# Giuseppe5/brevitas

Measured on AMD Instinct MI355X. Metric: Gelem/s fused int8 fake-quant fwd+bwd, per-channel, [256,512,56,56], higher is better.
Workload: dtype bf16

## Files before the change

brevitas_amd/csrc/bvq_fakequant.h:

```cpp
#pragma once

#include "bvq_quant_math.h"
#include "bvq_unit_walk.h"
#include "bvq_ties.h"
#include "bvq_sums.h"

namespace bvq {

struct QuantArgs {
  Tiling t;
  const void* x;
  const void* scale;
  const void* zp;
  void* y;
  void* codes;
  const void* g;
  float* ds_part;
  float* dzp_part;
  float* dq_part;
  const float* bounds;
  const void* tie_stat;
  unsigned long long* tie_info;
  unsigned long long* pos_part;
  float qmin, qmax;
  int32_t scale_dtype, zp_dtype;
  int32_t scale_pc, zp_pc;
  int32_t scalar_cast;
  int32_t clamp_ste;
  int32_t out_int;
  int32_t round_mode;
  int32_t pre_relu;
  int32_t codes_dtype;
  uint32_t* arrive;
  uint32_t arrive_per_channel;
  float* dscale_out;
  int32_t gs_scale_dtype, gs_quot_dtype;
  float gs_int_threshold;
  double* shard_msg;
  long long* shard_pos;
  int32_t shard_rank;
  int32_t pre_act;
};

#ifndef BVQ_FWD_UNROLL
#define BVQ_FWD_UNROLL 8
#endif
#ifndef BVQ_BWD_WAVES
#define BVQ_BWD_WAVES 4
#endif
#ifndef BVQ_F16_BWD_DIV
#define BVQ_F16_BWD_DIV 1
#endif
#ifndef BVQ_F16_BWD_PIPE
#define BVQ_F16_BWD_PIPE 1
#endif
#ifndef BVQ_F16_COLS_DIV
#define BVQ_F16_COLS_DIV 1
#endif
#ifndef BVQ_BWD_DEPTH
#define BVQ_BWD_DEPTH 4
#endif
constexpr int kUnroll = BVQ_FWD_UNROLL;
constexpr int kBwdDepth = BVQ_BWD_DEPTH;

template <typename CT>
__device__ __forceinline__ void load_scale_zp(const QuantArgs& a, int32_t channel, float& s, float& z) {
  s = load_scalar_as_f(a.scale, a.scale_dtype, a.scale_pc ? channel : 0);
  z = load_scalar_as_f(a.zp, a.zp_dtype, a.zp_pc ? channel : 0);
  if (a.scalar_cast) {
    if (!a.scale_pc) s = rnd<CT>(s);
    if (!a.zp_pc) z = rnd<CT>(z);
  }
}

template <typename CT, int RM>
__device__ __forceinline__ float do_round(float t, int mode) {
  if constexpr (RM == kAnyRM) {
    return round_any<CT>(t, mode);
  } else {
    return round_op<CT, RM>(t);
  }
}
template <typename CT, int RM>
__device__ __forceinline__ f2 do_round2(f2 t, int mode) {
  if constexpr (RM == kAnyRM) {
    return round_any2<CT>(t, mode);
  } else {
    return round_op2<CT, RM>(t);
  }
}
__device__ __forceinline__ f2 relu2(f2 v) {
  const f2 zero = splat2(0.f);
  return v < zero ? zero : v;
}

struct DivExact {
  float s;
  __device__ __forceinline__ float operator()(float a) const { return a / s; }
  __device__ __forceinline__ f2 operator()(f2 a) const {
    f2 r = {a.x / s, a.y / s};
    return r;
  }
};
struct DivBf16 {
  float r;
  __device__ __forceinline__ float operator()(float a) const { return a * r; }
  __device__ __forceinline__ f2 operator()(f2 a) const { return a * r; }
};

struct DivExactV {
  f2 s;
  __device__ __forceinline__ f2 operator()(f2 a) const {
    f2 r = {a.x / s.x, a.y / s.y};
    return r;
  }
};
struct DivBf16V {
  f2 r;
  __device__ __forceinline__ f2 operator()(f2 a) const { return a * r; }
};

__device__ __forceinline__ bool f16_quot_small(float q) {
  return (__builtin_bit_cast(uint32_t, q) & 0x7fffffffu) - 1u < 0x38810000u - 1u;
}
struct DivF16 {
  float s, r;
  __device__ __forceinline__ float operator()(float a) const {
    float q = a * r;
    if (__builtin_amdgcn_ballot_w64(f16_quot_small(q)) != 0) q = a / s;
    return q;
  }
  __device__ __forceinline__ f2 operator()(f2 a) const {
    f2 q = a * r;
    if (__builtin_amdgcn_ballot_w64(f16_quot_small(q.x) || f16_quot_small(q.y)) != 0) {
      q.x = a.x / s;
      q.y = a.y / s;
    }
    return q;
  }
};
struct DivF16V {
  f2 s, r;
  __device__ __forceinline__ f2 operator()(f2 a) const {
    f2 q = a * r;
    if (__builtin_amdgcn_ballot_w64(f16_quot_small(q.x) || f16_quot_small(q.y)) != 0) {
      q.x = a.x / s.x;
      q.y = a.y / s.y;
    }
    return q;
  }
};
__device__ __forceinline__ float div_refined(float a, float s, float r) {
  const float q0 = a * r;
  const float rem = __builtin_fmaf(-q0, s, a);
  return __builtin_amdgcn_div_fixupf(__builtin_fmaf(rem, r, q0), s, a);
}
struct DivF16R {
  float s, r;
  __device__ __forceinline__ float operator()(float a) const { return div_refined(a, s, r); }
  __device__ __forceinline__ f2 operator()(f2 a) const {
    f2 q = {div_refined(a.x, s, r), div_refined(a.y, s, r)};
    return q;
  }
};
#if BVQ_F16_COLS_DIV
#define BVQ_DIVF16V DivF16RV
#else
#define BVQ_DIVF16V DivF16V
#endif
struct DivF16RV {
  f2 s, r;
  __device__ __forceinline__ f2 operator()(f2 a) const {
    f2 q = {div_refined(a.x, s.x, r.x), div_refined(a.y, s.y, r.y)};
    return q;
  }
};
__device__ __forceinline__ bool f16_scale_ok(float s) {
  const uint32_t sb = __builtin_bit_cast(uint32_t, s);
  return (sb & 0x1fffu) == 0u && s >= 6.103515625e-05f && s <= 16384.f;
}

__device__ __forceinline__ bool bf16_scale_ok(float s) {
  const uint32_t sb = __builtin_bit_cast(uint32_t, s);
  return (sb & 0xffffu) == 0u && s >= 6.103515625e-05f && s <= 16384.f;
}
__device__ __forceinline__ bool zp_is_pos_zero(float z) { return __builtin_bit_cast(uint32_t, z) == 0u; }

struct ColsQuantArgs {
  ColsPlan p;
  const void* x;
  const void* g;
  void* y;
  const void* scale;
  const void* zp;
  float* ds_part;
  unsigned long long* pos_part;
  const void* tie_stat;
  unsigned long long* tie_info;
  int64_t inner;
  int32_t channels;
  float qmin, qmax;
  int32_t scale_dtype, zp_dtype, zp_pc, scalar_cast, clamp_ste, round_mode, pre_relu;
};

template <typename T, int V = elem<T>::vec>
struct ColsLane : ColsPlace {
  static constexpr int VEC = V;
  int32_t ch[VEC];
  f2 s2[VEC / 2], z2[VEC / 2];
  bool fast, zp0;

  __device__ __forceinline__ bool init(const ColsQuantArgs& a, bool team = false) {
    if (!cols_locate(a.p, team, *this)) return false;
    bool ok_fast = true, ok_zp0 = true;
    float sv[VEC], zv[VEC];
#pragma unroll
    for (int k = 0; k < VEC; ++k) {
      const int64_t col = active ? (int64_t)chunk * VEC + k : 0;
      ch[k] = (int32_t)(col / a.inner);
      sv[k] = load_scalar_as_f(a.scale, a.scale_dtype, ch[k]);
      zv[k] = load_scalar_as_f(a.zp, a.zp_dtype, a.zp_pc ? ch[k] : 0);
      if (a.scalar_cast && !a.zp_pc) zv[k] = rnd<T>(zv[k]);
      ok_fast = ok_fast && (elem<T>::id == BVQ_F16 ? f16_scale_ok(sv[k]) : bf16_scale_ok(sv[k]));
      ok_zp0 = ok_zp0 && zp_is_pos_zero(zv[k]);
    }
#pragma unroll
    for (int k = 0; k < VEC / 2; ++k) {
      s2[k] = f2{sv[2 * k], sv[2 * k + 1]};
      z2[k] = f2{zv[2 * k], zv[2 * k + 1]};
    }
    fast = sizeof(T) == 2 && __builtin_amdgcn_ballot_w64(!ok_fast) == 0;
    zp0 = sizeof(T) == 2 && __builtin_amdgcn_ballot_w64(!ok_zp0) == 0;
    return true;
  }
};


static int validate(const bvq_quant_desc* d, bool act = false) {
  if (!d) {
    set_error("null descriptor");
    return BVQ_ERR_INVALID;
  }
  if (d->outer < 0 || d->channels < 1 || d->inner < 0) {
    set_error("bad shape [%lld,%lld,%lld]", (long long)d->outer, (long long)d->channels,
              (long long)d->inner);
    return BVQ_ERR_INVALID;
  }
// ... 97 lines not shown
```

brevitas_amd/csrc/bvq_fakequant_fwd.hip:

```cpp

#include "bvq_act.h"
#include "bvq_fakequant.h"
#include "bvq_stat_epilogue.h"

namespace bvq {

template <typename CT, int RM, bool ZP0, typename Div>
__device__ __forceinline__ float fwd_elem(float xf, const Div& div, float s, float z, float qmin,
                                          float qmax, bool out_int, int mode, float& q_out) {
  float t = rnd<CT>(div(xf));
  t = ZP0 ? t + 0.f : rnd<CT>(t + z);
  t = do_round<CT, RM>(t, mode);
  const float q = clamp_where(t, qmin, qmax);
  q_out = q;
  if (out_int) return q;
  return ZP0 ? rnd<CT>(q * s) : rnd<CT>(rnd<CT>(q - z) * s);
}

template <typename CT, int RM, bool ZP0, typename Div, typename S>
__device__ __forceinline__ f2 fwd_elem2(f2 xf, const Div& div, S s, S z, float qmin, float qmax,
                                        bool out_int, int mode, f2& q_out) {
  f2 t = rnd2<CT>(div(xf));
  t = ZP0 ? t + 0.f : rnd2<CT>(t + z);
  t = do_round2<CT, RM>(t, mode);
  const f2 q = clamp_where2(t, qmin, qmax);
  q_out = q;
  if (out_int) return q;
  return ZP0 ? q * s : rnd2<CT>(q - z) * s;
}

template <int VEC>
__device__ __forceinline__ void store_codes(void* base, int codes_dtype, int64_t off, const float* q) {
  if (codes_dtype == BVQ_CODES_I32) {
    vec_t<int32_t, VEC> cv;
#pragma unroll
    for (int k = 0; k < VEC; ++k) cv.v[k] = (int32_t)q[k];
    store_vec<int32_t, VEC>(reinterpret_cast<int32_t*>(base) + off, cv);
  } else if (codes_dtype == BVQ_CODES_I8) {
    vec_t<int8_t, VEC> cv;
#pragma unroll
    for (int k = 0; k < VEC; ++k) cv.v[k] = (int8_t)(int32_t)q[k];
    store_vec<int8_t, VEC>(reinterpret_cast<int8_t*>(base) + off, cv);
  } else {
    vec_t<uint8_t, VEC> cv;
#pragma unroll
    for (int k = 0; k < VEC; ++k) cv.v[k] = (uint8_t)(int32_t)q[k];
    store_vec<uint8_t, VEC>(reinterpret_cast<uint8_t*>(base) + off, cv);
  }
}

template <typename XT, typename CT, int VEC, int RM, bool NT, bool ZP0, bool PRE, bool NTL = NT, int ACT = 0,
          typename Div>
__device__ __forceinline__ void fwd_unit(const QuantArgs& a, const Unit& u, const Div& div, float s,
                                         float z, float qmin, float qmax) {
  const int lane = threadIdx.x & 63;
  const XT* __restrict__ xp = reinterpret_cast<const XT*>(a.x) + u.base;
  CT* __restrict__ yp = a.y ? reinterpret_cast<CT*>(a.y) + u.base : nullptr;
  void* const cp = a.codes;
  const bool out_int = a.out_int != 0;
  const int mode = a.round_mode;

  ChunkCursor cur;
  cur.init(u, VEC, lane);
  const int64_t total = (int64_t)u.nrows * cur.cpr;
  for (int64_t done = 0; done < total; done += (int64_t)kWave * kUnroll) {
    vec_t<XT, VEC> xv[kUnroll];
    int64_t off[kUnroll];
    bool ok[kUnroll];
#pragma unroll
    for (int j = 0; j < kUnroll; ++j) {
      ok[j] = cur.valid();
      off[j] = cur.offset(u.row_stride, VEC);
      xv[j] = load_vec<XT, VEC, NTL>(xp + (ok[j] ? off[j] : 0));
      cur.next();
    }
#pragma unroll
    for (int j = 0; j < kUnroll; ++j) {
      if (ok[j]) {
        vec_t<CT, VEC> yv;
        float qv[VEC];
        if constexpr (VEC % 2 == 0) {
#pragma unroll
          for (int k = 0; k < VEC; k += 2) {
            f2 xf = widen2<XT>(xv[j].v[k], xv[j].v[k + 1]);
            if constexpr (PRE) xf = relu2(xf);
            if constexpr (ACT != 0) xf = act_rnd2<XT, ACT>(xf);
            f2 q2;
            const f2 r = fwd_elem2<CT, RM, ZP0>(xf, div, s, z, qmin, qmax, out_int, mode, q2);
            pack2<CT>(r, yv.v[k], yv.v[k + 1]);
            qv[k] = q2.x;
            qv[k + 1] = q2.y;
          }
        } else {
#pragma unroll
          for (int k = 0; k < VEC; ++k) {
            float xf = PRE ? relu_f(to_f<XT>(xv[j].v[k])) : to_f<XT>(xv[j].v[k]);
            if constexpr (ACT != 0) xf = act_rnd<XT, ACT>(xf);
            const float r = fwd_elem<CT, RM, ZP0>(xf, div, s, z, qmin, qmax, out_int, mode, qv[k]);
            yv.v[k] = from_f<CT>(r);
          }
        }
        if (yp) store_vec<CT, VEC, NT>(yp + off[j], yv);
        if (cp) store_codes<VEC>(cp, a.codes_dtype, u.base + off[j], qv);
      }
    }
  }
  const int32_t tail = (int32_t)(u.len - (int64_t)cur.cpr * VEC);
  for (int32_t e = lane; e < u.nrows * tail; e += kWave) {
    const int32_t tr = e / tail, tk = e - tr * tail;
    const int64_t i = (int64_t)tr * u.row_stride + (int64_t)cur.cpr * VEC + tk;
    float q;
    float xf = PRE ? relu_f(to_f<XT>(xp[i])) : to_f<XT>(xp[i]);
    if constexpr (ACT != 0) xf = act_rnd<XT, ACT>(xf);
    const float r = fwd_elem<CT, RM, ZP0>(xf, div, s, z, qmin, qmax, out_int, mode, q);
    if (yp) yp[i] = from_f<CT>(r);
    if (cp) store_codes<1>(cp, a.codes_dtype, u.base + i, &q);
  }
}

template <typename XT, typename CT, int VEC, int RM, bool NT, bool NTL = NT, int ACT = 0>
__global__ __launch_bounds__(kBlock) void fakequant_fwd_kernel(QuantArgs a) {
  const Unit u = locate_unit(a.t);
  if (!u.valid) return;
  float s, z;
  load_scale_zp<CT>(a, u.channel, s, z);
  const float qmin = rnd<CT>(a.bounds ? a.bounds[0] : a.qmin), qmax = rnd<CT>(a.bounds ? a.bounds[1] : a.qmax);
  const bool zp0 = sizeof(CT) == 2 && zp_is_pos_zero(z);
#define BVQ_FWD_UNIT(ZP0, PRE, DIV) fwd_unit<XT, CT, VEC, RM, NT, ZP0, PRE, NTL, ACT>(a, u, DIV, s, z, qmin, qmax)
#define BVQ_FWD_PRE(ZP0, DIV)      \
  do {                             \
    if constexpr (ACT != 0)        \
      BVQ_FWD_UNIT(ZP0, false, DIV); \
    else if (a.pre_relu)           \
      BVQ_FWD_UNIT(ZP0, true, DIV); \
    else                           \
      BVQ_FWD_UNIT(ZP0, false, DIV); \
  } while (0)
  if constexpr (elem<CT>::id == BVQ_BF16) {
    if (bf16_scale_ok(s)) {
      const DivBf16 div{1.0f / s};
      if (zp0)
        BVQ_FWD_PRE(true, div);
      else
        BVQ_FWD_PRE(false, div);
      return;
    }
  }
#ifndef BVQ_F16_FWD_EXACT
  if constexpr (elem<CT>::id == BVQ_F16) {
    if (f16_scale_ok(s)) {
      const DivF16R div{s, 1.0f / s};
      if (zp0)
        BVQ_FWD_PRE(true, div);
      else
        BVQ_FWD_PRE(false, div);
      return;
    }
  }
#endif
  const DivExact div{s};
  if constexpr (sizeof(CT) == 2) {
    if (zp0) {
      BVQ_FWD_PRE(true, div);
      return;
    }
  }
  BVQ_FWD_PRE(false, div);
#undef BVQ_FWD_PRE
#undef BVQ_FWD_UNIT
}


template <typename T>
constexpr int kColsFwdVec = sizeof(T) == 2 ? kColsFwdVec16 : elem<T>::vec;

template <typename T, int RM, bool NT, bool ZP0, bool FAST, bool PRE>
__device__ __forceinline__ void cols_fwd_rows(const ColsQuantArgs& a, const ColsLane<T, kColsFwdVec<T>>& ln, float qmin,
                                              float qmax) {
  constexpr int VEC = kColsFwdVec<T>;
#ifndef BVQ_COLS_FWD_UNROLL
#define BVQ_COLS_FWD_UNROLL 4
#endif
  constexpr int kU = BVQ_COLS_FWD_UNROLL;
  const int64_t nrows = ln.row_end - ln.blk0;
  const uint32_t bytes = (uint32_t)(nrows * a.p.L * (int64_t)sizeof(T));
  const buf_t bx = make_buf(reinterpret_cast<const T*>(a.x) + ln.blk0 * a.p.L, bytes);
  const buf_t by = make_buf(reinterpret_cast<T*>(a.y) + ln.blk0 * a.p.L, bytes);
  const uint32_t step = (uint32_t)((int64_t)a.p.rpp * a.p.L * (int64_t)sizeof(T));
  uint32_t off = (uint32_t)(((int64_t)ln.sub * a.p.L + (int64_t)ln.chunk * VEC) * (int64_t)sizeof(T));
  const int32_t steps = (int32_t)((nrows + a.p.rpp - 1) / a.p.rpp);
  f2 r2[VEC / 2];
#pragma unroll
  for (int k = 0; k < VEC / 2; ++k) r2[k] = f2{1.0f / ln.s2[k].x, 1.0f / ln.s2[k].y};
  const int mode = a.round_mode;
  for (int32_t i = 0; i < steps; i += kU) {
    vec_t<T, VEC> xv[kU];
#pragma unroll
    for (int j = 0; j < kU; ++j) xv[j] = buf_load<T, VEC, NT>(bx, off + (uint32_t)j * step);
#pragma unroll
    for (int j = 0; j < kU; ++j) {
      if (i + j < steps) {
        vec_t<T, VEC> yv;
#pragma unroll
        for (int k = 0; k < VEC; k += 2) {
          f2 xf = widen2<T>(xv[j].v[k], xv[j].v[k + 1]);
          if constexpr (PRE) xf = relu2(xf);
          f2 q2, res;
          if constexpr (FAST && elem<T>::id == BVQ_F16)
            res = fwd_elem2<T, RM, ZP0>(xf, BVQ_DIVF16V{ln.s2[k / 2], r2[k / 2]}, ln.s2[k / 2], ln.z2[k / 2], qmin, qmax, false,
                                        mode, q2);
          else if constexpr (FAST)
            res = fwd_elem2<T, RM, ZP0>(xf, DivBf16V{r2[k / 2]}, ln.s2[k / 2], ln.z2[k / 2], qmin, qmax, false, mode, q2);
          else
            res = fwd_elem2<T, RM, ZP0>(xf, DivExactV{ln.s2[k / 2]}, ln.s2[k / 2], ln.z2[k / 2], qmin, qmax, false, mode, q2);
          pack2<T>(res, yv.v[k], yv.v[k + 1]);
        }
        buf_store<T, VEC, NT>(by, off + (uint32_t)j * step, yv);
      }
    }
    off += (uint32_t)kU * step;
  }
}

template <typename T, int RM, bool NT>
__global__ __launch_bounds__(kBlock) void fakequant_fwd_cols_kernel(ColsQuantArgs a) {
  ColsLane<T, kColsFwdVec<T>> ln;
  if (!ln.init(a) || !ln.active) return;
  const float qmin = rnd<T>(a.qmin), qmax = rnd<T>(a.qmax);
#define BVQ_COLS_FWD(ZP0, FAST)                                \
  do {                                                         \
    if (a.pre_relu)                                            \
      cols_fwd_rows<T, RM, NT, ZP0, FAST, true>(a, ln, qmin, qmax);  \
    else                                                       \
      cols_fwd_rows<T, RM, NT, ZP0, FAST, false>(a, ln, qmin, qmax); \
  } while (0)
  if constexpr (sizeof(T) == 2) {
    if (ln.fast) {
      if (ln.zp0)
        BVQ_COLS_FWD(true, true);
      else
        BVQ_COLS_FWD(false, true);
      return;
    }
    if (ln.zp0) {
      BVQ_COLS_FWD(true, false);
      return;
    }
  }
  BVQ_COLS_FWD(false, false);
#undef BVQ_COLS_FWD
}

constexpr int kFusedSlots = 8;
constexpr int kFusedSliceChunks = 512;
constexpr int kFusedMaxWaves = 8;

struct FusedArgs {
  const void* x;
  void* y;
  void* stat_out;
  void* scale_out;
  int64_t outer, inner;
  int32_t channels;
  int32_t cpr;
  int32_t spr;
  int32_t slices;
  float qmin, qmax, min_val, int_threshold;
  int32_t use_min, scale_dtype, scale_pc, scalar_cast, round_mode, pre_relu;
};

template <typename T>
__device__ __forceinline__ float scale_from_key(uint32_t key, bool use_min, float min_val, float int_threshold,
                                                int scale_dtype, float& stat) {
  if constexpr (elem<T>::id == BVQ_F16)
    stat = (float)__builtin_bit_cast(f16_t, (uint16_t)key);
  else
    stat = __builtin_bit_cast(float, key);
  const float thr = (use_min && stat < min_val) ? min_val : stat;
  float s = thr / int_threshold;
  if (scale_dtype == BVQ_BF16)
    s = rnd<bf16_t>(s);
  else if (scale_dtype == BVQ_F16)
    s = rnd<f16_t>(s);
  return s;
}
template <typename T>
__device__ __forceinline__ void store_stat_scale(void* stat_out, void* scale_out, int scale_dtype, int32_t c,
                                                 float stat, float s) {
  if constexpr (elem<T>::id == BVQ_F32)
    reinterpret_cast<float*>(stat_out)[c] = stat;
  else
    reinterpret_cast<T*>(stat_out)[c] = (T)stat;
  if (scale_dtype == BVQ_F32)
    reinterpret_cast<float*>(scale_out)[c] = s;
  else if (scale_dtype == BVQ_BF16)
    reinterpret_cast<bf16_t*>(scale_out)[c] = (bf16_t)s;
  else
    reinterpret_cast<f16_t*>(scale_out)[c] = (f16_t)s;
}

template <typename T, int RM, bool PRE, typename Div, typename Ok>
__device__ __forceinline__ void fused_quantize(const vec_t<T, elem<T>::vec> (&xv)[kFusedSlots], const Ok& ok,
                                               T* __restrict__ yp, int lane, const Div& div, float s,
                                               float qmin, float qmax, int mode) {
  constexpr int VEC = elem<T>::vec;
  constexpr bool ZP0 = sizeof(T) == 2;
#pragma unroll
  for (int j = 0; j < kFusedSlots; ++j) {
    if (ok[j]) {
      vec_t<T, VEC> yv;
#pragma unroll
      for (int k = 0; k < VEC; k += 2) {
        f2 xf = widen2<T>(xv[j].v[k], xv[j].v[k + 1]);
        if constexpr (PRE) xf = relu2(xf);
        f2 q2;
        const f2 r = fwd_elem2<T, RM, ZP0>(xf, div, s, 0.f, qmin, qmax, false, mode, q2);
        pack2<T>(r, yv.v[k], yv.v[k + 1]);
      }
      store_vec<T, VEC, true>(yp + (int64_t)(lane + kWave * j) * VEC, yv);
    }
  }
}

__global__ void fused_zero_kernel(uint32_t* p, int64_t n) {
  const int64_t i = (int64_t)blockIdx.x * blockDim.x + threadIdx.x;
  if (i < n) p[i] = 0u;
}

__device__ __forceinline__ void fused_slice(const FusedArgs& a, int q, int lane, int& r, int& sl, bool (&ok)[kFusedSlots]) {
  const bool active = q < a.slices;
  r = active ? q / a.spr : 0;
  sl = active ? q - r * a.spr : 0;
  const int nch = active ? (a.cpr - sl * kFusedSliceChunks < kFusedSliceChunks ? a.cpr - sl * kFusedSliceChunks
                                                                              : kFusedSliceChunks)
                         : 0;
#pragma unroll
  for (int j = 0; j < kFusedSlots; ++j) ok[j] = lane + kWave * j < nch;
}

template <typename T>
__device__ __forceinline__ void fused_load(const FusedArgs& a, int32_t c, int r, int sl, const bool (&ok)[kFusedSlots],
                                           int lane, vec_t<T, elem<T>::vec> (&xv)[kFusedSlots]) {
  constexpr int VEC = elem<T>::vec;
  const int64_t base = ((int64_t)r * a.channels + c) * a.inner + (int64_t)sl * kFusedSliceChunks * VEC;
  const T* __restrict__ xp = reinterpret_cast<const T*>(a.x) + base;
#pragma unroll
  for (int j = 0; j < kFusedSlots; ++j)
    xv[j] = load_vec<T, VEC, true>(ok[j] ? xp + (int64_t)(lane + kWave * j) * VEC : reinterpret_cast<const T*>(a.x));
}

struct SlotCount {
  int lane, nch;
  __device__ __forceinline__ bool operator[](int j) const { return lane + kWave * j < nch; }
};
__device__ __forceinline__ void fused_slice(const FusedArgs& a, int q, int lane, int& r, int& sl, SlotCount& ok) {
  const bool active = q < a.slices;
  r = active ? q / a.spr : 0;
  sl = active ? q - r * a.spr : 0;
  const int left = a.cpr - sl * kFusedSliceChunks;
  ok.lane = lane;
  ok.nch = active ? (left < kFusedSliceChunks ? left : kFusedSliceChunks) : 0;
}
template <typename T>
__device__ __forceinline__ void fused_load(const FusedArgs& a, int32_t c, int r, int sl, const SlotCount& ok, int lane,
                                           vec_t<T, elem<T>::vec> (&xv)[kFusedSlots]) {
  constexpr int VEC = elem<T>::vec;
  const int64_t base = ((int64_t)r * a.channels + c) * a.inner + (int64_t)sl * kFusedSliceChunks * VEC;
  const T* __restrict__ xp = reinterpret_cast<const T*>(a.x) + base;
  asm volatile("" : "+v"(lane));
#pragma unroll
  for (int j = 0; j < kFusedSlots; ++j)
    xv[j] = load_vec<T, VEC, true>(xp + (lane + kWave * j < ok.nch ? (uint32_t)(lane + kWave * j) * VEC : 0u));
}

template <typename T, typename Ok>
__device__ __forceinline__ uint32_t fused_key(const FusedArgs& a, const vec_t<T, elem<T>::vec> (&xv)[kFusedSlots],
                                              const Ok& ok) {
  uint32_t m = 0;
#pragma unroll
  for (int j = 0; j < kFusedSlots; ++j) {
    if (ok[j]) {
#pragma unroll
      for (int k = 0; k < elem<T>::vec; ++k) {
        const uint32_t b = a.pre_relu ? pre_abs_bits<T, true>(xv[j].v[k]) : pre_abs_bits<T, false>(xv[j].v[k]);
        m = b > m ? b : m;
      }
    }
  }
  return m;
}
template <typename T, std::enable_if_t<sizeof(T) == 4, int> = 0>
__device__ __forceinline__ uint32_t fused_key(const FusedArgs& a, const vec_t<T, elem<T>::vec> (&xv)[kFusedSlots],
                                              const SlotCount& ok) {
  uint32_t m = 0;
#pragma unroll
  for (int j = 0; j < kFusedSlots; ++j) {
    uint32_t mj = 0;
#pragma unroll
    for (int k = 0; k < elem<T>::vec; ++k) {
      const uint32_t b = a.pre_relu ? pre_abs_bits<T, true>(xv[j].v[k]) : pre_abs_bits<T, false>(xv[j].v[k]);
      mj = b > mj ? b : mj;
    }
    mj = ok[j] ? mj : 0u;
    m = mj > m ? mj : m;
  }
  return m;
}

template <typename T, int RM, typename Ok>
__device__ __forceinline__ void fused_apply(const FusedArgs& a, int32_t c, int r, int sl,
                                            const vec_t<T, elem<T>::vec> (&xv)[kFusedSlots], const Ok& ok,
                                            float s, float qmin, float qmax, int lane) {
  constexpr int VEC = elem<T>::vec;
  const int64_t base = ((int64_t)r * a.channels + c) * a.inner + (int64_t)sl * kFusedSliceChunks * VEC;
  T* __restrict__ yp = reinterpret_cast<T*>(a.y) + base;
  const int mode = a.round_mode;
  if constexpr (elem<T>::id == BVQ_BF16) {
    if (bf16_scale_ok(s)) {
      const DivBf16 div{1.0f / s};
      if (a.pre_relu)
        fused_quantize<T, RM, true>(xv, ok, yp, lane, div, s, qmin, qmax, mode);
      else
        fused_quantize<T, RM, false>(xv, ok, yp, lane, div, s, qmin, qmax, mode);
      return;
    }
  }
  if constexpr (elem<T>::id == BVQ_F16) {
    if (f16_scale_ok(s)) {
      const DivF16R div{s, 1.0f / s};
      if (a.pre_relu)
        fused_quantize<T, RM, true>(xv, ok, yp, lane, div, s, qmin, qmax, mode);
      else
        fused_quantize<T, RM, false>(xv, ok, yp, lane, div, s, qmin, qmax, mode);
      return;
    }
  }
  const DivExact div{s};
  if (a.pre_relu)
    fused_quantize<T, RM, true>(xv, ok, yp, lane, div, s, qmin, qmax, mode);
  else
    fused_quantize<T, RM, false>(xv, ok, yp, lane, div, s, qmin, qmax, mode);
}

template <typename T, int RM>
__device__ __forceinline__ void fused_channel(const FusedArgs& a, int32_t c, int r, int sl, const bool (&ok)[kFusedSlots],
                                              float qmin, float qmax, int wave, int lane, int nwaves,
                                              uint32_t* sh_max, uint32_t& sh_stat) {
  vec_t<T, elem<T>::vec> xv[kFusedSlots];
  fused_load<T>(a, c, r, sl, ok, lane, xv);
  const uint32_t m = wave_max_u32(fused_key<T>(a, xv, ok));
  if (lane == 0) sh_max[wave] = m;
  __syncthreads();
  if (threadIdx.x == 0) {
    uint32_t bm = 0;
    for (int w = 0; w < nwaves; ++w) bm = sh_max[w] > bm ? sh_max[w] : bm;
    sh_stat = bm;
  }
  __syncthreads();
  float stat;
  float s = scale_from_key<T>(sh_stat, a.use_min, a.min_val, a.int_threshold, a.scale_dtype, stat);
  if (threadIdx.x == 0) store_stat_scale<T>(a.stat_out, a.scale_out, a.scale_dtype, c, stat, s);
  if (a.scalar_cast && !a.scale_pc) s = rnd<T>(s);
  fused_apply<T, RM>(a, c, r, sl, xv, ok, s, qmin, qmax, lane);
}

template <typename T, int RM>
__global__ __launch_bounds__(kFusedMaxWaves * kWave) void fused_absmax_fakequant_kernel(FusedArgs a) {
  __shared__ uint32_t sh_max[kFusedMaxWaves];
  __shared__ uint32_t sh_stat;
  const int lane = threadIdx.x & 63;
  const int wave = __builtin_amdgcn_readfirstlane((int)(threadIdx.x >> 6));
  const int nwaves = (int)(blockDim.x >> 6);
  int r, sl;
  bool ok[kFusedSlots];
  fused_slice(a, wave, lane, r, sl, ok);
  const float qmin = rnd<T>(a.qmin), qmax = rnd<T>(a.qmax);
  for (int32_t c = blockIdx.x; c < a.channels; c += gridDim.x)
    fused_channel<T, RM>(a, c, r, sl, ok, qmin, qmax, wave, lane, nwaves, sh_max, sh_stat);
}

struct FusedListArgs {
  FusedArgs a[BVQ_WEIGHT_LIST_MAX];
  int32_t start[BVQ_WEIGHT_LIST_MAX + 1];
  int32_t n;
};
static_assert(sizeof(FusedListArgs) <= 4096, "kernel arguments are limited to 4 KiB");

template <typename T, int RM>
__global__ __launch_bounds__(kFusedMaxWaves * kWave) void fused_list_fakequant_kernel(FusedListArgs la) {
  __shared__ uint32_t sh_max[kFusedMaxWaves];
  __shared__ uint32_t sh_stat;
  const int lane = threadIdx.x & 63;
  const int wave = __builtin_amdgcn_readfirstlane((int)(threadIdx.x >> 6));
  const int nwaves = (int)(blockDim.x >> 6);
  int p = -1, r = 0, sl = 0;
  bool ok[kFusedSlots];
  float qmin = 0.f, qmax = 0.f;
  for (int32_t pair = blockIdx.x; pair < la.start[la.n]; pair += gridDim.x) {
    if (p < 0 || pair >= la.start[p + 1]) {
      if (p < 0) p = 0;
      while (p + 1 < la.n && pair >= la.start[p + 1]) ++p;
      fused_slice(la.a[p], wave, lane, r, sl, ok);
      qmin = rnd<T>(la.a[p].qmin);
      qmax = rnd<T>(la.a[p].qmax);
    }
    fused_channel<T, RM>(la.a[p], pair - la.start[p], r, sl, ok, qmin, qmax, wave, lane, nwaves, sh_max, sh_stat);
  }
}


constexpr int kClusterWaves = 16;
constexpr int kClusterMaxMembers = kWave;
constexpr uint32_t kClusterTag = 0x80000000u;
constexpr uint64_t kClusterBudgetTicks = 200000;
enum { kClusterAuto = 0, kClusterWalk = 1, kClusterOneShot = 2 };

struct ClusterArgs {
  FusedArgs f;
  ScaleEpilogue ep;
  void* stat_out;
  int32_t in_dtype;
  uint32_t* key;
  uint32_t* dep;
  uint32_t* fallbacks;
  int32_t members, nclusters, force_fallback;
#ifdef BVQ_CLUSTER_STAMPS
  uint64_t* stamps;
#endif
};

constexpr int kClusterStamps = 6;
#ifdef BVQ_CLUSTER_STAMPS
#define BVQ_CLUSTER_STAMP(k) \
  do {                       \
    if (wave == 0) tk[k] = __builtin_amdgcn_s_memrealtime(); \
  } while (0)
#else
#define BVQ_CLUSTER_STAMP(k) \
  do {                       \
  } while (0)
#endif

__device__ __forceinline__ uint32_t cluster_wave_max(uint32_t v) {
#define BVQ_DPP_MAX(ctrl)                                                                       \
  do {                                                                                          \
    const uint32_t o = (uint32_t)__builtin_amdgcn_update_dpp(0, (int)v, ctrl, 0xf, 0xf, false); \
    v = o > v ? o : v;                                                                          \
  } while (0)
  BVQ_DPP_MAX(0xB1);
  BVQ_DPP_MAX(0x4E);
  BVQ_DPP_MAX(0x141);
  BVQ_DPP_MAX(0x140);
#undef BVQ_DPP_MAX
  const uint32_t a = (uint32_t)__builtin_amdgcn_readlane((int)v, 0), b = (uint32_t)__builtin_amdgcn_readlane((int)v, 16);
  const uint32_t c = (uint32_t)__builtin_amdgcn_readlane((int)v, 32), d = (uint32_t)__builtin_amdgcn_readlane((int)v, 48);
  const uint32_t ab = a > b ? a : b, cd = c > d ? c : d;
  return ab > cd ? ab : cd;
}

template <typename T>
__device__ __forceinline__ uint32_t cluster_fallback_key(const FusedArgs& a, int32_t c, int wave, int lane) {
  constexpr int VEC = elem<T>::vec;
  uint32_t fm = 0;
  for (int q = wave; q < a.slices; q += kClusterWaves) {
    const int fr = q / a.spr, fsl = q - fr * a.spr;
    const int left = a.cpr - fsl * kFusedSliceChunks;
    const int nch = left < kFusedSliceChunks ? left : kFusedSliceChunks;
    const T* xp = reinterpret_cast<const T*>(a.x) + ((int64_t)fr * a.channels + c) * a.inner +
                  (int64_t)fsl * kFusedSliceChunks * VEC;
#pragma clang loop unroll(disable)
    for (int i = lane; i < nch; i += kWave) {
      const vec_t<T, VEC> u = load_vec<T, VEC, false>(xp + (int64_t)i * VEC);
#pragma unroll
      for (int k = 0; k < VEC; ++k) {
        const uint32_t b = a.pre_relu ? pre_abs_bits<T, true>(u.v[k]) : pre_abs_bits<T, false>(u.v[k]);
        fm = b > fm ? b : fm;
      }
    }
  }
  return cluster_wave_max(fm);
}

template <typename T, int RM>
__global__ __launch_bounds__(kClusterWaves * kWave, 8) void cluster_absmax_fakequant_kernel(ClusterArgs ca) {
  constexpr int VEC = elem<T>::vec;
  __shared__ uint32_t sh_max[kClusterWaves];
  __shared__ uint32_t sh_stat, sh_ok;
  const FusedArgs& a = ca.f;
  const int lane = threadIdx.x & 63;
  const int wave = __builtin_amdgcn_readfirstlane((int)(threadIdx.x >> 6));
  const int32_t members = ca.members;
  const int32_t member = (int32_t)blockIdx.x % members, cluster = (int32_t)blockIdx.x / members;
  int r, sl;
  SlotCount ok;
  fused_slice(a, member * kClusterWaves + wave, lane, r, sl, ok);
  const float qmin = rnd<T>(a.qmin), qmax = rnd<T>(a.qmax);
  int32_t c = cluster;
  if (c >= a.channels) return;
#ifdef BVQ_CLUSTER_STAMPS
  uint64_t tk[kClusterStamps] = {};
#endif
  BVQ_CLUSTER_STAMP(0);
  vec_t<T, VEC> xv[kFusedSlots];
  fused_load<T>(a, c, r, sl, ok, lane, xv);
  for (; c < a.channels; c += ca.nclusters) {
    const uint32_t m = cluster_wave_max(fused_key<T>(a, xv, ok));
    if (lane == 0) sh_max[wave] = m;
    BVQ_CLUSTER_STAMP(1);
    __syncthreads();
    uint32_t* const keys = ca.key + (int64_t)c * members;
    if (wave == 0) {
      uint32_t bm = 0;
      for (int w = 0; w < kClusterWaves; ++w) bm = sh_max[w] > bm ? sh_max[w] : bm;
      if (lane == 0) __hip_atomic_store(keys + member, bm | kClusterTag, __ATOMIC_RELAXED, __HIP_MEMORY_SCOPE_AGENT);
    }
    BVQ_CLUSTER_STAMP(2);
    const int32_t cn = c + ca.nclusters;
    if (wave == 0) {
      bool done = false;
      uint32_t v = 0;
      if (!ca.force_fallback) {
        const uint64_t t0 = __builtin_amdgcn_s_memrealtime();
        for (;;) {
          v = lane < members ? __hip_atomic_load(keys + lane, __ATOMIC_RELAXED, __HIP_MEMORY_SCOPE_AGENT) : kClusterTag;
          if (__all((v & kClusterTag) != 0)) {
            done = true;
            break;
          }
          if (__builtin_amdgcn_s_memrealtime() - t0 > kClusterBudgetTicks) break;
          __builtin_amdgcn_s_sleep(2);
        }
      }
      v = cluster_wave_max(v) & ~kClusterTag;
      if (lane == 0) {
        sh_stat = v;
        sh_ok = done ? 1u : 0u;
      }
    }
    __syncthreads();
    if (!sh_ok) {
      const uint32_t fm = cluster_fallback_key<T>(a, c, wave, lane);
      if (lane == 0) sh_max[wave] = fm;
      __syncthreads();
      if (threadIdx.x == 0) {
        uint32_t bm = 0;
        for (int w = 0; w < kClusterWaves; ++w) bm = sh_max[w] > bm ? sh_max[w] : bm;
        sh_stat = bm;
        if (ca.fallbacks) __hip_atomic_fetch_add(ca.fallbacks, 1u, __ATOMIC_RELAXED, __HIP_MEMORY_SCOPE_AGENT);
      }
      __syncthreads();
    }
    BVQ_CLUSTER_STAMP(3);
    const uint32_t key = sh_stat;
    uint32_t before = 0;
    if (wave == 0) {
      if (lane == 0) {
        if (!sh_ok) asm volatile("s_waitcnt vmcnt(0)" ::: "memory");
        before = __hip_atomic_fetch_add(ca.dep + c, 1u, __ATOMIC_RELAXED, __HIP_MEMORY_SCOPE_AGENT);
      }
    }
    float stat;
    const float s = scale_from_key<T>(key, a.use_min, a.min_val, a.int_threshold, a.scale_dtype, stat);
    if (member == 0 && threadIdx.x == 0) absmax_epilogue(ca.stat_out, ca.in_dtype, ca.in_dtype, ca.ep, c, key);
    if constexpr (RM == kAnyRM && elem<T>::id == BVQ_BF16) {
      switch (a.round_mode) {
#define BVQ_CLUSTER_APPLY(M)                                              \
  case M:                                                                 \
    fused_apply<T, M>(a, c, r, sl, xv, ok, s, qmin, qmax, lane); \
    break
        BVQ_CLUSTER_APPLY(BVQ_ROUND);
        BVQ_CLUSTER_APPLY(BVQ_FLOOR);
        BVQ_CLUSTER_APPLY(BVQ_CEIL);
        BVQ_CLUSTER_APPLY(BVQ_ROUND_TO_ZERO);
        default:
          fused_apply<T, BVQ_DPU_ROUND>(a, c, r, sl, xv, ok, s, qmin, qmax, lane);
#undef BVQ_CLUSTER_APPLY
      }
    } else {
      fused_apply<T, RM>(a, c, r, sl, xv, ok, s, qmin, qmax, lane);
    }
    BVQ_CLUSTER_STAMP(4);
    if (wave == 0) {
      before = __builtin_amdgcn_readfirstlane(before);
      if (before + 1 == (uint32_t)members) {
        if (lane < members) __hip_atomic_store(keys + lane, 0u, __ATOMIC_RELAXED, __HIP_MEMORY_SCOPE_AGENT);
        if (lane == 0) __hip_atomic_store(ca.dep + c, 0u, __ATOMIC_RELAXED, __HIP_MEMORY_SCOPE_AGENT);
      }
    }
#ifdef BVQ_CLUSTER_STAMPS
    BVQ_CLUSTER_STAMP(5);
    if (ca.stamps && wave == 0 && lane < kClusterStamps) {
      uint64_t t = tk[0];
#pragma unroll
      for (int k = 1; k < kClusterStamps; ++k) t = lane == k ? tk[k] : t;
      ca.stamps[((int64_t)c * members + member) * kClusterStamps + lane] = t;
    }
    if (wave == 0) tk[0] = tk[5];
#endif
    if (cn < a.channels) fused_load<T>(a, cn, r, sl, ok, lane, xv);
  }
}
#undef BVQ_CLUSTER_STAMP

}

using namespace bvq;

static int fakequant_fwd_impl(const bvq_quant_desc* d, const void* x, const void* scale, const void* zp, void* y,
                             void* codes, const float* bounds, bvq_stream_t stream) {
  int rc = validate(d, true);
  if (rc) return rc;
  const bool act = d->pre_op >= BVQ_PRE_SIGMOID;
  if (act && (codes || bounds || !y || d->out_kind != BVQ_OUT_DEQUANT || d->x_dtype != d->ct_dtype)) {
    set_error("bvq_fakequant_fwd: pre_op %d needs the dequantized output in x's dtype, no codes, no device bounds",
              d->pre_op);
    return BVQ_ERR_UNSUPPORTED;
  }
  const int64_t n = d->outer * d->channels * d->inner;
  if (n == 0) return BVQ_OK;
  if (!x || !scale || !zp || (!y && !codes)) {
    set_error("bvq_fakequant_fwd: null pointer");
    return BVQ_ERR_INVALID;
  }
  if (y && !codes && !bounds && !act) {
    const ColsPlan cp = cols_quant_plan(d, x, y, nullptr, true, false, kColsFwdVec16);
    if (cp.ok) {
      ColsQuantArgs ca = {};
      fill_cols_args(ca, cp, d);
      ca.x = x;
      ca.y = y;
      ca.scale = scale;
      ca.zp = zp;
      hipStream_t cst = (hipStream_t)stream;
      const bool cnt = n * (int64_t)(2 * dtype_size(d->x_dtype)) >= nt_threshold_bytes();
      rc = with_cols_variant(d, cnt, [&](auto t, auto rm, auto ntc) {
        fakequant_fwd_cols_kernel<typename decltype(t)::type, rm, ntc><<<grid_for_units(cp.units), kBlock, 0, cst>>>(ca);
      });
      return rc ? rc : check_launch("bvq_fakequant_fwd/cols");
    }
  }
  int64_t outer, row_len;
  int32_t channels;
  rows_of(d, outer, row_len, channels);
  const void* ptrs[3] = {x, y, codes};
  const int els[3] = {dtype_size(d->x_dtype), dtype_size(d->ct_dtype), d->codes_dtype == BVQ_CODES_I32 ? 4 : 1};
  const int full = 16 / dtype_size(d->x_dtype);
  const int vec = snap_vec(pick_vec(full, outer * channels, row_len, ptrs, els, 3, true), full);
  QuantArgs a = {};
  a.t = make_tiling(outer, channels, row_len, vec, 0, true);
  a.x = x;
  a.scale = scale;
  a.zp = zp;
  a.y = y;
  a.codes = codes;
  a.bounds = bounds;
  fill_args(a, d);
  hipStream_t st = (hipStream_t)stream;
  const bool nt = n * (int64_t)(dtype_size(d->x_dtype) + dtype_size(d->ct_dtype)) >= nt_threshold_bytes();
  if (act) {
    rc = with_dtype(d->x_dtype, [&](auto xt) {
      using XT = typename decltype(xt)::type;
      return with_value<BVQ_PRE_SIGMOID, BVQ_PRE_TANH>(d->pre_op, [&](auto ac) {
        return with_stream_variant<elem<XT>::vec>("bvq_fakequant_fwd", vec, a.round_mode, nt, [&](auto v, auto rm, auto ntc) {
          fakequant_fwd_kernel<XT, XT, v, rm, ntc, ntc, ac><<<grid_for_units(a.t.units), kBlock, 0, st>>>(a);
        });
      });
    });
    return rc ? rc : check_launch("bvq_fakequant_fwd");
  }
  rc = with_pair(d->x_dtype, d->ct_dtype, [&](auto xt, auto ct) {
    using XT = typename decltype(xt)::type;
    return with_stream_variant<elem<XT>::vec>("bvq_fakequant_fwd", vec, a.round_mode, nt, [&](auto v, auto rm, auto ntc) {
      fakequant_fwd_kernel<XT, typename decltype(ct)::type, v, rm, ntc><<<grid_for_units(a.t.units), kBlock, 0, st>>>(a);
    });
  });
  return rc ? rc : check_launch("bvq_fakequant_fwd");
}

extern "C" int bvq_fakequant_fwd(const bvq_quant_desc* d, const void* x, const void* scale,
                                 const void* zp, void* y, void* codes, bvq_stream_t stream) {
  return fakequant_fwd_impl(d, x, scale, zp, y, codes, nullptr, stream);
}

extern "C" int bvq_fakequant_fwd_bounds(const bvq_quant_desc* d, const void* x, const void* scale, const void* zp,
                                        const float* bounds, void* y, bvq_stream_t stream) {
  if (!bounds) {
    set_error("bvq_fakequant_fwd_bounds: null bounds");
    return BVQ_ERR_INVALID;
  }
  return fakequant_fwd_impl(d, x, scale, zp, y, nullptr, bounds, stream);
}


struct FusedPlan {
  int32_t cpr, spr, slices, waves, nblocks;
};

static int num_cus() {
  static int n = [] {
    int dev = 0, v = 0;
    if (hipGetDevice(&dev) != hipSuccess ||
        hipDeviceGetAttribute(&v, hipDeviceAttributeMultiprocessorCount, dev) != hipSuccess || v <= 0)
      v = 256;
    return v;
  }();
  return n;
}

struct FusedShape {
  bool ok;
  int64_t outer, channels, inner;
  int vec;
};

#ifndef BVQ_FUSED_FWD
#define BVQ_FUSED_FWD 1
#endif
// ... 299 lines not shown
```

brevitas_amd/csrc/bvq_quant_math.h:

```cpp
#pragma once

#include "bvq_common.h"

namespace bvq {

template <typename CT, int RM>
__device__ __forceinline__ float round_op(float t) {
  if constexpr (RM == BVQ_ROUND) {
    return __builtin_rintf(t);
  } else if constexpr (RM == BVQ_FLOOR) {
    return __builtin_floorf(t);
  } else if constexpr (RM == BVQ_CEIL) {
    return __builtin_ceilf(t);
  } else if constexpr (RM == BVQ_ROUND_TO_ZERO) {
    float sg = (float)(0.f < t) - (float)(t < 0.f);
    return sg * __builtin_floorf(__builtin_fabsf(t));
  } else {
    float fr = rnd<CT>(t - __builtin_floorf(t));
    return (t < 0.f && fr == 0.5f) ? __builtin_ceilf(t) : __builtin_rintf(t);
  }
}

template <typename CT>
__device__ __forceinline__ float round_any(float t, int mode) {
  switch (mode) {
    case BVQ_ROUND:
      return round_op<CT, BVQ_ROUND>(t);
    case BVQ_FLOOR:
      return round_op<CT, BVQ_FLOOR>(t);
    case BVQ_CEIL:
      return round_op<CT, BVQ_CEIL>(t);
    case BVQ_ROUND_TO_ZERO:
      return round_op<CT, BVQ_ROUND_TO_ZERO>(t);
    default:
      return round_op<CT, BVQ_DPU_ROUND>(t);
  }
}

__device__ __forceinline__ float clamp_where(float t, float qmin, float qmax) {
  t = t > qmax ? qmax : t;
  t = t < qmin ? qmin : t;
  return t;
}

typedef float f2 __attribute__((ext_vector_type(2)));
typedef int b2 __attribute__((ext_vector_type(2)));

template <typename T>
__device__ __forceinline__ f2 rnd2(f2 v) {
  f2 r = {rnd<T>(v.x), rnd<T>(v.y)};
  return r;
}
template <>
__device__ __forceinline__ f2 rnd2<float>(f2 v) {
  return v;
}
template <>
__device__ __forceinline__ f2 rnd2<bf16_t>(f2 v) {
  typedef bf16_t bf16x2 __attribute__((ext_vector_type(2)));
  const uint32_t bits = __builtin_bit_cast(uint32_t, __builtin_convertvector(v, bf16x2));
  f2 r = {__builtin_bit_cast(float, bits << 16), __builtin_bit_cast(float, bits & 0xffff0000u)};
  return r;
}

template <>
__device__ __forceinline__ f2 rnd2<f16_t>(f2 v) {
  typedef f16_t f16x2 __attribute__((ext_vector_type(2)));
  float a = v.x, b = v.y;
  asm volatile("" : "+v"(a), "+v"(b));
  f2 w = {a, b};
  return __builtin_convertvector(__builtin_convertvector(w, f16x2), f2);
}

template <typename T>
__device__ __forceinline__ void pack2(f2 v, T& a, T& b) {
  a = from_f<T>(v.x);
  b = from_f<T>(v.y);
}
template <>
__device__ __forceinline__ void pack2<bf16_t>(f2 v, bf16_t& a, bf16_t& b) {
  typedef bf16_t bf16x2 __attribute__((ext_vector_type(2)));
  const bf16x2 h = __builtin_convertvector(v, bf16x2);
  a = h.x;
  b = h.y;
}

template <>
__device__ __forceinline__ void pack2<f16_t>(f2 v, f16_t& a, f16_t& b) {
  typedef f16_t f16x2 __attribute__((ext_vector_type(2)));
  float x = v.x, y = v.y;
  asm volatile("" : "+v"(x), "+v"(y));
  f2 w = {x, y};
  const f16x2 h = __builtin_convertvector(w, f16x2);
  a = h.x;
  b = h.y;
}

template <typename T>
__device__ __forceinline__ f2 widen2(T a, T b) {
  f2 r = {to_f<T>(a), to_f<T>(b)};
  return r;
}

__device__ __forceinline__ f2 splat2(float v) {
  f2 r = {v, v};
  return r;
}

template <typename CT, int RM>
__device__ __forceinline__ f2 round_op2(f2 t) {
  if constexpr (RM == BVQ_ROUND) {
    return __builtin_elementwise_roundeven(t);
  } else if constexpr (RM == BVQ_FLOOR) {
    return __builtin_elementwise_floor(t);
  } else if constexpr (RM == BVQ_CEIL) {
    return __builtin_elementwise_ceil(t);
  } else {
    f2 r = {round_op<CT, RM>(t.x), round_op<CT, RM>(t.y)};
    return r;
  }
}

template <typename CT>
__device__ __forceinline__ f2 round_any2(f2 t, int mode) {
  switch (mode) {
    case BVQ_ROUND:
      return round_op2<CT, BVQ_ROUND>(t);
    case BVQ_FLOOR:
      return round_op2<CT, BVQ_FLOOR>(t);
    case BVQ_CEIL:
      return round_op2<CT, BVQ_CEIL>(t);
    case BVQ_ROUND_TO_ZERO:
      return round_op2<CT, BVQ_ROUND_TO_ZERO>(t);
    default:
      return round_op2<CT, BVQ_DPU_ROUND>(t);
  }
}

__device__ __forceinline__ f2 clamp_where2(f2 t, float qmin, float qmax) {
  const f2 hi = splat2(qmax), lo = splat2(qmin);
  t = t > hi ? hi : t;
  t = t < lo ? lo : t;
  return t;
}

}
```

Measured before the change: 577.8.

## Add lean fused quantize path with med3 clamp, bitwise relu, and packed absmax fold

When the scale and clamp bounds are well-formed, the fused quantize uses a leaner per-element path: relu is applied bitwise on packed 16-bit values, zero-point handling is dropped, and clamping uses fmed3. The absmax key reduction is rewritten to fold packed 16-bit lanes with elementwise integer max, with explicit NaN handling for the relu case. The cluster round-mode dispatch is also extended from bf16 to all 2-byte types. The goal is fewer VALU instructions per element in a kernel that is expected to be close to memory-bound, at the cost of extra template instantiations and possible subtle differences in NaN and edge-case semantics.

```diff
diff --git a/brevitas_amd/csrc/bvq_fakequant.h b/brevitas_amd/csrc/bvq_fakequant.h
--- a/brevitas_amd/csrc/bvq_fakequant.h
+++ b/brevitas_amd/csrc/bvq_fakequant.h
@@ -93,6 +93,22 @@
   const f2 zero = splat2(0.f);
   return v < zero ? zero : v;
 }
+template <typename T, int VEC>
+__device__ __forceinline__ vec_t<T, VEC> relu_bits(const vec_t<T, VEC>& v) {
+  if constexpr (sizeof(T) == 2) {
+    typedef short i16x2 __attribute__((ext_vector_type(2)));
+    vec_t<uint32_t, VEC / 2> w = __builtin_bit_cast(vec_t<uint32_t, VEC / 2>, v);
+#pragma unroll
+    for (int k = 0; k < VEC / 2; ++k)
+      w.v[k] = __builtin_bit_cast(uint32_t, __builtin_elementwise_max(__builtin_bit_cast(i16x2, w.v[k]), i16x2{0, 0}));
+    return __builtin_bit_cast(vec_t<T, VEC>, w);
+  } else {
+    vec_t<int32_t, VEC> w = __builtin_bit_cast(vec_t<int32_t, VEC>, v);
+#pragma unroll
+    for (int k = 0; k < VEC; ++k) w.v[k] = w.v[k] > 0 ? w.v[k] : 0;
+    return __builtin_bit_cast(vec_t<T, VEC>, w);
+  }
+}
 
 struct DivExact {
   float s;
diff --git a/brevitas_amd/csrc/bvq_fakequant_fwd.hip b/brevitas_amd/csrc/bvq_fakequant_fwd.hip
--- a/brevitas_amd/csrc/bvq_fakequant_fwd.hip
+++ b/brevitas_amd/csrc/bvq_fakequant_fwd.hip
@@ -27,6 +27,14 @@
   q_out = q;
   if (out_int) return q;
   return ZP0 ? q * s : rnd2<CT>(q - z) * s;
+}
+
+template <typename CT, int RM, bool NONNEG, typename Div>
+__device__ __forceinline__ f2 fwd_elem2_lean(f2 xf, const Div& div, float s, float qmin, float qmax, int mode) {
+  f2 t = rnd2<CT>(div(xf));
+  if constexpr (!NONNEG) t = t + 0.f;
+  t = do_round2<CT, RM>(t, mode);
+  return clamp_med3_2(t, qmin, qmax) * s;
 }
 
 template <int VEC>
@@ -299,7 +307,7 @@
     reinterpret_cast<f16_t*>(scale_out)[c] = (f16_t)s;
 }
 
-template <typename T, int RM, bool PRE, typename Div, typename Ok>
+template <typename T, int RM, bool PRE, bool LEAN, typename Div, typename Ok>
 __device__ __forceinline__ void fused_quantize(const vec_t<T, elem<T>::vec> (&xv)[kFusedSlots], const Ok& ok,
                                                T* __restrict__ yp, int lane, const Div& div, float s,
                                                float qmin, float qmax, int mode) {
@@ -309,13 +317,22 @@
   for (int j = 0; j < kFusedSlots; ++j) {
     if (ok[j]) {
       vec_t<T, VEC> yv;
-#pragma unroll
-      for (int k = 0; k < VEC; k += 2) {
-        f2 xf = widen2<T>(xv[j].v[k], xv[j].v[k + 1]);
-        if constexpr (PRE) xf = relu2(xf);
-        f2 q2;
-        const f2 r = fwd_elem2<T, RM, ZP0>(xf, div, s, 0.f, qmin, qmax, false, mode, q2);
-        pack2<T>(r, yv.v[k], yv.v[k + 1]);
+      if constexpr (LEAN) {
+        const vec_t<T, VEC> xr = PRE ? relu_bits<T, VEC>(xv[j]) : xv[j];
+#pragma unroll
+        for (int k = 0; k < VEC; k += 2) {
+          const f2 r = fwd_elem2_lean<T, RM, PRE>(widen2<T>(xr.v[k], xr.v[k + 1]), div, s, qmin, qmax, mode);
+          pack2<T>(r, yv.v[k], yv.v[k + 1]);
+        }
+      } else {
+#pragma unroll
+        for (int k = 0; k < VEC; k += 2) {
+          f2 xf = widen2<T>(xv[j].v[k], xv[j].v[k + 1]);
+          if constexpr (PRE) xf = relu2(xf);
+          f2 q2;
+          const f2 r = fwd_elem2<T, RM, ZP0>(xf, div, s, 0.f, qmin, qmax, false, mode, q2);
+          pack2<T>(r, yv.v[k], yv.v[k + 1]);
+        }
       }
       store_vec<T, VEC, true>(yp + (int64_t)(lane + kWave * j) * VEC, yv);
     }
@@ -346,7 +363,7 @@
   const T* __restrict__ xp = reinterpret_cast<const T*>(a.x) + base;
 #pragma unroll
   for (int j = 0; j < kFusedSlots; ++j)
-    xv[j] = load_vec<T, VEC, true>(ok[j] ? xp + (int64_t)(lane + kWave * j) * VEC : reinterpret_cast<const T*>(a.x));
+    xv[j] = load_vec<T, VEC, true>(ok[j] ? xp + (int64_t)(lane + kWave * j) * VEC : xp);
 }
 
 struct SlotCount {
@@ -373,38 +390,63 @@
     xv[j] = load_vec<T, VEC, true>(xp + (lane + kWave * j < ok.nch ? (uint32_t)(lane + kWave * j) * VEC : 0u));
 }
 
+template <typename T, bool PRE, typename Ok>
+__device__ __forceinline__ uint32_t fused_key_fold(const vec_t<T, elem<T>::vec> (&xv)[kFusedSlots], const Ok& ok) {
+  constexpr int VEC = elem<T>::vec;
+  if constexpr (sizeof(T) == 2) {
+    typedef unsigned short u16x2 __attribute__((ext_vector_type(2)));
+    typedef short i16x2 __attribute__((ext_vector_type(2)));
+    constexpr uint32_t kNegInf = elem<T>::id == BVQ_BF16 ? 0xff80u : 0xfc00u;
+    u16x2 um = {0, 0};
+    i16x2 sm = {0, 0};
+#pragma unroll
+    for (int j = 0; j < kFusedSlots; ++j) {
+      const vec_t<uint32_t, VEC / 2> w = __builtin_bit_cast(vec_t<uint32_t, VEC / 2>, xv[j]);
+#pragma unroll
+      for (int k = 0; k < VEC / 2; ++k) {
+        if constexpr (PRE) {
+          sm = __builtin_elementwise_max(sm, __builtin_bit_cast(i16x2, w.v[k]));
+          um = __builtin_elementwise_max(um, __builtin_bit_cast(u16x2, w.v[k]));
+        } else {
+          um = __builtin_elementwise_max(um, __builtin_bit_cast(u16x2, w.v[k] & 0x7fff7fffu));
+        }
+      }
+    }
+    uint32_t m16 = um.x > um.y ? um.x : um.y;
+    if constexpr (PRE) {
+      const uint32_t pos = (uint32_t)(sm.x > sm.y ? sm.x : sm.y);
+      const uint32_t nan = m16 > kNegInf ? (m16 & 0x7fffu) : 0u;
+      m16 = pos > nan ? pos : nan;
+    }
+    return elem<T>::id == BVQ_BF16 ? (m16 << 16) : m16;
+  } else {
+    uint32_t um = 0;
+    int32_t sm = 0;
+#pragma unroll
+    for (int j = 0; j < kFusedSlots; ++j) {
+#pragma unroll
+      for (int k = 0; k < VEC; ++k) {
+        const uint32_t w = ok[j] ? __builtin_bit_cast(uint32_t, xv[j].v[k]) : 0u;
+        if constexpr (PRE) {
+          sm = (int32_t)w > sm ? (int32_t)w : sm;
+          um = w > um ? w : um;
+        } else {
+          const uint32_t b = w & 0x7fffffffu;
+          um = b > um ? b : um;
+        }
+      }
+    }
+    if constexpr (PRE) {
+      const uint32_t nan = um > 0xff800000u ? (um & 0x7fffffffu) : 0u;
+      return (uint32_t)sm > nan ? (uint32_t)sm : nan;
+    }
+    return um;
+  }
+}
 template <typename T, typename Ok>
 __device__ __forceinline__ uint32_t fused_key(const FusedArgs& a, const vec_t<T, elem<T>::vec> (&xv)[kFusedSlots],
                                               const Ok& ok) {
-  uint32_t m = 0;
-#pragma unroll
-  for (int j = 0; j < kFusedSlots; ++j) {
-    if (ok[j]) {
-#pragma unroll
-      for (int k = 0; k < elem<T>::vec; ++k) {
-        const uint32_t b = a.pre_relu ? pre_abs_bits<T, true>(xv[j].v[k]) : pre_abs_bits<T, false>(xv[j].v[k]);
-        m = b > m ? b : m;
-      }
-    }
-  }
-  return m;
-}
-template <typename T, std::enable_if_t<sizeof(T) == 4, int> = 0>
-__device__ __forceinline__ uint32_t fused_key(const FusedArgs& a, const vec_t<T, elem<T>::vec> (&xv)[kFusedSlots],
-                                              const SlotCount& ok) {
-  uint32_t m = 0;
-#pragma unroll
-  for (int j = 0; j < kFusedSlots; ++j) {
-    uint32_t mj = 0;
-#pragma unroll
-    for (int k = 0; k < elem<T>::vec; ++k) {
-      const uint32_t b = a.pre_relu ? pre_abs_bits<T, true>(xv[j].v[k]) : pre_abs_bits<T, false>(xv[j].v[k]);
-      mj = b > mj ? b : mj;
-    }
-    mj = ok[j] ? mj : 0u;
-    m = mj > m ? mj : m;
-  }
-  return m;
+  return a.pre_relu ? fused_key_fold<T, true>(xv, ok) : fused_key_fold<T, false>(xv, ok);
 }
 
 template <typename T, int RM, typename Ok>
@@ -415,31 +457,38 @@
   const int64_t base = ((int64_t)r * a.channels + c) * a.inner + (int64_t)sl * kFusedSliceChunks * VEC;
   T* __restrict__ yp = reinterpret_cast<T*>(a.y) + base;
   const int mode = a.round_mode;
+  const bool pre = a.pre_relu != 0;
+  const bool lean = lean_clamp_ok(s, qmin, qmax, pre);
+#define BVQ_FUSED_QUANTIZE(DIV)                                                        \
+  do {                                                                                 \
+    if (lean) {                                                                        \
+      if (pre)                                                                         \
+        fused_quantize<T, RM, true, true>(xv, ok, yp, lane, DIV, s, qmin, qmax, mode);  \
+      else                                                                             \
+        fused_quantize<T, RM, false, true>(xv, ok, yp, lane, DIV, s, qmin, qmax, mode); \
+    } else if (pre) {                                                                  \
+      fused_quantize<T, RM, true, false>(xv, ok, yp, lane, DIV, s, qmin, qmax, mode);   \
+    } else {                                                                           \
+      fused_quantize<T, RM, false, false>(xv, ok, yp, lane, DIV, s, qmin, qmax, mode);  \
+    }                                                                                  \
+  } while (0)
   if constexpr (elem<T>::id == BVQ_BF16) {
     if (bf16_scale_ok(s)) {
       const DivBf16 div{1.0f / s};
-      if (a.pre_relu)
-        fused_quantize<T, RM, true>(xv, ok, yp, lane, div, s, qmin, qmax, mode);
-      else
-        fused_quantize<T, RM, false>(xv, ok, yp, lane, div, s, qmin, qmax, mode);
+      BVQ_FUSED_QUANTIZE(div);
       return;
     }
   }
   if constexpr (elem<T>::id == BVQ_F16) {
     if (f16_scale_ok(s)) {
       const DivF16R div{s, 1.0f / s};
-      if (a.pre_relu)
-        fused_quantize<T, RM, true>(xv, ok, yp, lane, div, s, qmin, qmax, mode);
-      else
-        fused_quantize<T, RM, false>(xv, ok, yp, lane, div, s, qmin, qmax, mode);
+      BVQ_FUSED_QUANTIZE(div);
       return;
     }
   }
   const DivExact div{s};
-  if (a.pre_relu)
-    fused_quantize<T, RM, true>(xv, ok, yp, lane, div, s, qmin, qmax, mode);
-  else
-    fused_quantize<T, RM, false>(xv, ok, yp, lane, div, s, qmin, qmax, mode);
+  BVQ_FUSED_QUANTIZE(div);
+#undef BVQ_FUSED_QUANTIZE
 }
 
 template <typename T, int RM>
@@ -662,7 +711,7 @@
     float stat;
     const float s = scale_from_key<T>(key, a.use_min, a.min_val, a.int_threshold, a.scale_dtype, stat);
     if (member == 0 && threadIdx.x == 0) absmax_epilogue(ca.stat_out, ca.in_dtype, ca.in_dtype, ca.ep, c, key);
-    if constexpr (RM == kAnyRM && elem<T>::id == BVQ_BF16) {
+    if constexpr (RM == kAnyRM && sizeof(T) == 2) {
       switch (a.round_mode) {
 #define BVQ_CLUSTER_APPLY(M)                                              \
   case M:                                                                 \
diff --git a/brevitas_amd/csrc/bvq_quant_math.h b/brevitas_amd/csrc/bvq_quant_math.h
--- a/brevitas_amd/csrc/bvq_quant_math.h
+++ b/brevitas_amd/csrc/bvq_quant_math.h
@@ -144,4 +144,12 @@
   return t;
 }
 
+__device__ __forceinline__ f2 clamp_med3_2(f2 t, float qmin, float qmax) {
+  f2 r = {__builtin_amdgcn_fmed3f(t.x, qmin, qmax), __builtin_amdgcn_fmed3f(t.y, qmin, qmax)};
+  return r;
 }
+__device__ __forceinline__ bool lean_clamp_ok(float s, float qmin, float qmax, bool pre_relu) {
+  return s > 0.f && s < __builtin_inff() && qmin <= qmax && qmax != 0.f && (pre_relu || qmin != 0.f);
+}
+
+}
```

Measured after the change: 584.5, median of 6. 1.01x the previous value.
